# architector1324/micro-raytracer

Hardware: AMD Instinct MI355X
Metric: Msamples/sec (res x spp) (higher is better)
Workload: dtype f32

## Files before the change

### micro_raytracer_amd/csrc/mrt_pack.cpp

```cpp
#include "mrt_pack.h"

#include <math.h>
#include <stdarg.h>
#include <stdio.h>
#include <string.h>

#include <algorithm>
#include <map>
#include <array>

namespace mrt {
namespace {

constexpr u32 kBvhMinInstances = 24;

struct H3 { float x, y, z; };
inline H3 h3(float x, float y, float z) { H3 r = {x, y, z}; return r; }
inline H3 hadd(H3 a, H3 b) { return h3(a.x + b.x, a.y + b.y, a.z + b.z); }
inline H3 hsub(H3 a, H3 b) { return h3(a.x - b.x, a.y - b.y, a.z - b.z); }
inline H3 hmuls(H3 a, float s) { return h3(a.x * s, a.y * s, a.z * s); }
inline H3 hneg(H3 a) { return h3(-a.x, -a.y, -a.z); }
inline H3 hhadam(H3 a, H3 b) { return h3(a.x * b.x, a.y * b.y, a.z * b.z); }
inline float hdot(H3 a, H3 b) { return a.x * b.x + a.y * b.y + a.z * b.z; }
inline H3 hcross(H3 a, H3 b) { return h3(a.y * b.z - a.z * b.y, a.z * b.x - a.x * b.z, a.x * b.y - a.y * b.x); }
// ... 683 lines not shown
    if (!ident) {
        double M[9];
        for (int a = 0; a < 3; ++a) for (int b2 = 0; b2 < 3; ++b2) { double acc = 0; for (int k = 0; k < 3; ++k) acc += (double)X[XF_R + a * 3 + k] * X[XF_L + k * 3 + b2]; M[a * 3 + b2] = acc; }
        for (int a = 0; a < 3 && ortho; ++a) for (int b2 = 0; b2 < 3; ++b2) { double acc = 0; for (int k = 0; k < 3; ++k) acc += M[a * 3 + k] * M[b2 * 3 + k]; if (!(fabs(acc - (a == b2 ? 1.0 : 0.0)) < 1e-4)) ortho = false; }
        for (int a = 0; a < 3; ++a) { lo[a] = -rad; hi[a] = rad; }
    }
    const double pp[3] = {pos.x, pos.y, pos.z};
    bd.ok = ortho && rad < 1e6;
    for (int a = 0; a < 3 && bd.ok; ++a) {
        const double slack = 1e-3 * fmax(fabs(lo[a]), fabs(hi[a])) + 1e-6;
        bd.mn[a] = (float)(pp[a] + lo[a] - slack); bd.mx[a] = (float)(pp[a] + hi[a] + slack);
        if (!(fabs(pp[a]) < 1e6) || !(bd.mn[a] <= bd.mx[a])) bd.ok = false;
    }
    return bd;
}

int add_instance(const mrt_renderer &o, u32 r, const mrt_instance &in, Tables &T, std::string &err)
{
    u32 ir[INST_WORDS] = {0};
    u32 ix[INSTX_WORDS] = {0};
    const H3 pos = h3(in.pos[0], in.pos[1], in.pos[2]);
    put3(ir + INST_POS, pos);
    const u32 xf = T.xf_of(in.dir);
    if ((unsigned long long)xf * XF_WORDS >= (1ull << 28)) return reject(err, MRT_ERR_LIMIT, "too many distinct instance directions");
    const float *X = T.xf_tab.data() + (size_t)xf * XF_WORDS;
    ir[INST_TAG] = o.kind | (bits(X[XF_IDENT]) ? TAG_IDENT : 0u) | ((xf * XF_WORDS) << TAG_XF_SHIFT);
    ix[INSTX_REND] = r;
    const u32 *geo = &T.rend_tab[(size_t)r * REND_WORDS + REND_GEO];
    if (o.kind == MRT_KIND_SPHERE) {
        ir[INST_P3] = geo[0];
    } else if (o.kind == MRT_KIND_PLANE) {
        const H3 nn = h3(fbits(geo[0]), fbits(geo[1]), fbits(geo[2])), nraw = h3(fbits(geo[3]), fbits(geo[4]), fbits(geo[5]));
        ir[INST_P3] = bits(hdot(hneg(nn), pos));
        ir[INST_P5] = geo[0]; ir[INST_P5 + 1] = geo[1]; ir[INST_P5 + 2] = geo[2];
        put3(ix + INSTX_PLANE_NW, hnorm(mul3(X + XF_R, mul3(X + XF_L, nraw))));
    } else if (o.kind == MRT_KIND_BOX) {
        ir[INST_P3] = geo[0]; ir[INST_P5] = geo[1]; ir[INST_P5 + 1] = geo[2];
    }
    T.inst_tab.insert(T.inst_tab.end(), ir, ir + INST_WORDS);
    T.instx_tab.insert(T.instx_tab.end(), ix, ix + INSTX_WORDS);
    const bool tri = o.kind == MRT_KIND_TRIANGLE;
    T.bounds.push_back(instance_bound(o.kind, o.param, tri ? o.param : o.tris, tri ? 3 : (size_t)o.n_tris * 3, X, pos));
    return MRT_OK;
}

bool build_inst_bvh(Tables &T)
{
    std::vector<u32> elig;
    for (u32 i = 0; i < T.n_inst(); ++i) (T.bounds[i].ok ? elig : T.lin_list).push_back(i);
    if (T.n_inst() < kBvhMinInstances || elig.size() < kBvhMinInstances / 2) { T.lin_list.clear(); return false; }
    std::vector<TriBox> ib(T.n_inst());
    for (u32 i : elig) for (int a = 0; a < 3; ++a) { const Bound &b = T.bounds[i]; ib[i].mn[a] = b.mn[a]; ib[i].mx[a] = b.mx[a]; ib[i].c[a] = 0.5f * b.mn[a] + 0.5f * b.mx[a]; }
    TbvhBuild build{ib, T.bvh_nodes, T.bvh_inst, MRT_IBVH_LEAF_MAX};
    build.make(elig, 0, elig.size());
    const u32 n_nodes = (u32)(T.bvh_nodes.size() / BVH_WORDS);
    for (u32 k = 0; k < n_nodes; ++k) { float *q = T.bvh_nodes.data() + (size_t)k * BVH_WORDS; if (bits(q[BVH_SKIP]) >= n_nodes) q[BVH_SKIP] = fbits(BVH_END); }
    return true;
}

bool all_ident(const Tables &T)
{
    bool all = T.n_inst() > 0;
    const u32 xf0 = all ? T.inst_tab[INST_TAG] >> TAG_XF_SHIFT : 0u;
    for (u32 i = 0; i < T.n_inst() && all; ++i) {
        const u32 tag = T.inst_tab[(size_t)i * INST_WORDS + INST_TAG];
        all = (tag & TAG_IDENT) != 0u && memcmp(&T.xf_tab[tag >> TAG_XF_SHIFT], &T.xf_tab[xf0], XF_IDENT * sizeof(float)) == 0;
    }
    return all;
}

bool axis_table(Tables &T, bool plain_ident)
{
    bool scan = plain_ident;
    for (u32 i = 0; i < T.n_inst() && scan; ++i) {
        const u32 *ir = &T.inst_tab[(size_t)i * INST_WORDS];
        const u32 kind = ir[INST_TAG] & TAG_KIND_MASK;
        auto bounded = [](u32 w) { return fabsf(fbits(w)) <= kAxisMax; };
        u32 code = 0u, sd = 0u;
        bool ok = bounded(ir[INST_POS]) && bounded(ir[INST_POS + 1]) && bounded(ir[INST_POS + 2]) && bounded(ir[INST_P3]);
        if (kind == KIND_PLANE) {
            u32 ones = 0u, zeros = 0u;
            for (u32 k = 0; k < 3u; ++k) {
                const u32 w = ir[INST_P5 + k], mag = w & 0x7fffffffu;
                if (mag == 0x3f800000u) { ++ones; code = k + 1u; sd = ir[INST_P3] ^ (w & 0x80000000u); }
                else if (mag == 0u) ++zeros;
            }
            ok = ok && ones == 1u && zeros == 2u;
        } else if (kind != KIND_SPHERE) ok = false;
        T.axis_tab.push_back(code); T.axis_tab.push_back(sd);
        scan = ok;
    }
    return scan;
}

void inst_margins(const Tables &T, Params &P)
{
    float r_min = 3.0e38f;
    bool sphere = false;
    for (u32 i : T.bvh_inst) {
        if ((T.inst_tab[(size_t)i * INST_WORDS + INST_TAG] & TAG_KIND_MASK) != KIND_SPHERE) continue;
        sphere = true;
        for (int a = 0; a < 3; ++a) r_min = std::min(r_min, 0.5f * (T.bounds[i].mx[a] - T.bounds[i].mn[a]));
    }
    P.inst_k = 1e-4f;
    P.inst_ksq = !sphere ? 0.0f : (r_min > 1e-12f ? 4e-6f / r_min : 1e30f);
    P.inst_kpos = sphere ? 1e-5f : 2e-6f;
}

int check_lights(const mrt_scene &sc, std::string &err)
{
    for (u32 l = 0; l < sc.n_light; ++l) if (sc.light[l].kind > MRT_LIGHT_DIR) return reject(err, MRT_ERR_SCENE, "unknown light kind");
    return MRT_OK;
}

int level_order_wide(Tables &T, std::string &err)
{
    struct Ref { u32 depth, mesh, local; };
    std::vector<Ref> order;
    std::vector<std::vector<u32>> newi(T.wide.size());
    for (size_t m = 0; m < T.wide.size(); ++m) { newi[m].resize(T.wide[m].size()); for (size_t k = 0; k < T.wide[m].size(); ++k) order.push_back({T.wide[m][k].depth, (u32)m, (u32)k}); }
    std::stable_sort(order.begin(), order.end(), [](const Ref &a, const Ref &b) { return a.depth < b.depth; });
    if (order.size() >= (1u << 24)) return reject(err, MRT_ERR_LIMIT, "triangle BVHs too large");
    for (size_t k = 0; k < order.size(); ++k) newi[order[k].mesh][order[k].local] = (u32)k;
    T.tbvh_tab.assign(order.size() * B4_WORDS, 0.0f);
    for (size_t k = 0; k < order.size(); ++k) {
        const Wide4 &w = T.wide[order[k].mesh][order[k].local];
        float *q = T.tbvh_tab.data() + k * B4_WORDS;
        for (int c = 0; c < 4; ++c) {
            q[B4_CX + c] = w.c[c][0]; q[B4_CY + c] = w.c[c][1]; q[B4_CZ + c] = w.c[c][2];
            q[B4_HX + c] = w.h[c][0]; q[B4_HY + c] = w.h[c][1]; q[B4_HZ + c] = w.h[c][2];
            u32 cw = w.child[c];
            if (cw & B4_INTERNAL) cw = B4_INTERNAL | newi[order[k].mesh][cw & ~B4_INTERNAL];
            q[B4_CHILD + c] = fbits(cw);
        }
    }
    for (size_t m = 0; m < T.wide.size(); ++m) T.mesh_tab[(size_t)T.wide_mesh[m] * MESH_WORDS + MESH_TBVH] = newi[m][0];
    return MRT_OK;
}

int emit(const mrt_scene &sc, const mrt_env *env, const Tables &T, Packed &out, std::string &err)
{
    Params &P = out.P;
    Blob B;
    P.n_rend = sc.n_renderer; P.n_inst = T.n_inst(); P.n_light = sc.n_light;
    P.n_lin = (u32)T.lin_list.size(); P.n_bvh_nodes = (u32)(T.bvh_nodes.size() / BVH_WORDS);
    out.n_lin = P.n_lin; out.n_bvh_nodes = P.n_bvh_nodes;
    P.off_rend = B.table(T.rend_tab);
    P.off_cam = B.align4(); B.put(P.cam_L, 9); B.put(P.cam_R, 9);
    P.off_lin = B.table(T.lin_list);
    P.off_bvh = B.table(T.bvh_nodes);
    P.off_bvhinst = B.table(T.bvh_inst);
    P.off_inst = B.table(T.inst_tab);
    P.off_instx = B.table(T.instx_tab);
    P.off_axis = 0u; P.axis_scan = out.axis_scan ? 1u : 0u;
    if (out.axis_scan) P.off_axis = B.table(T.axis_tab);
    P.off_xf = B.table(T.xf_tab);
    P.off_mat = B.table(T.mat_tab);
    P.off_light = B.align4();
    for (u32 l = 0; l < sc.n_light; ++l) {
        const mrt_light &li = sc.light[l];
        B.u(li.kind);
        if (li.kind == MRT_LIGHT_POINT) B.f3(h3(li.v[0], li.v[1], li.v[2]));
        else B.f3(hnorm(hneg(hnorm(h3(li.v[0], li.v[1], li.v[2])))));
        B.f(li.pwr);
        B.f3(h3(li.color[0], li.color[1], li.color[2]));
    }
    P.off_tex = B.align4();
    B.w.resize(B.w.size() + (size_t)sc.n_textures * TEX_WORDS, 0);
    P.off_lut = B.align4();
    for (int k = 0; k < 256; ++k) B.f((float)k / 255.0f);
    P.off_mesh = B.table(T.mesh_tab);
    P.off_node = B.table(T.node_tab);
    P.off_parent = B.table(T.parent_tab);
    P.off_tbvh = B.table(T.tbvh_tab);
// ... 86 lines not shown
```

### micro_raytracer_amd/csrc/mrt_scene.h

```cpp
#pragma once
#include <stddef.h>

#include "mrt_math.h"

namespace mrt {

constexpr u32 REND_WORDS = 16;
constexpr u32 INST_WORDS = 8;
constexpr u32 XF_WORDS = 20;
constexpr u32 MAT_WORDS = 16;
constexpr u32 LIGHT_WORDS = 8;
constexpr u32 TEX_WORDS = 4;
constexpr u32 MESH_WORDS = 12;
constexpr u32 TRI_WORDS = 9;
constexpr u32 NODE_WORDS = 8;

enum : u32 { REND_KIND = 0, REND_INST_OFF = 1, REND_INST_CNT = 2, REND_FLAGS = 3, REND_GEO = 4 };
enum : u32 { RF_HAS_MAPS = 1u, RF_HAS_UV = 2u, RF_HAS_VN = 4u };
enum : u32 { REND_VATTR = 15 };
constexpr u32 VATTR_WORDS = 16;
enum : u32 { VATTR_VN = 0, VATTR_UV = 9 };

enum : u32 { INST_POS = 0, INST_P3 = 3, INST_TAG = 4, INST_P5 = 5 };
enum : u32 { INSTX_REND = 0, INSTX_PLANE_NW = 1 };
constexpr u32 INSTX_WORDS = 4;
enum : u32 { AXIS_CODE = 0, AXIS_SD = 1 };
constexpr u32 AXIS_WORDS = 2;
constexpr float kAxisMax = 0x1p38f;
constexpr u32 TAG_KIND_MASK = 7u, TAG_IDENT = 8u, TAG_XF_SHIFT = 4u;

enum : u32 { XF_L = 0, XF_R = 9, XF_IDENT = 18 };

enum : u32 { MAT_ALBEDO = 0, MAT_ROUGH = 3, MAT_METAL = 4, MAT_GLASS = 5, MAT_OPACITY = 6, MAT_EMIT = 7, MAT_MAP = 8, MAT_FLAGS = 14 };
enum : u32 { MATF_BILINEAR = 1u, MATF_CLAMP_V = 2u };
enum : u32 { MAP_TEX = 0, MAP_ROUGH = 1, MAP_METAL = 2, MAP_GLASS = 3, MAP_OPACITY = 4, MAP_EMIT = 5 };

enum : u32 { LIGHT_KIND = 0, LIGHT_V = 1, LIGHT_PWR = 4, LIGHT_COLOR = 5 };

enum : u32 { TEX_W = 0, TEX_H = 1, TEX_OFF = 2, TEX_FMT = 3 };
enum : u32 { TEXFMT_NONE = 0, TEXFMT_F32 = 1, TEXFMT_U8 = 2 };

enum : u32 { ENV_W = 0, ENV_H = 1, ENV_OFF = 2, ENV_FMT = 3, ENV_MAP = 4, ENV_ROT = 5, ENV_PWR = 6, ENV_FLAGS = 7 };
enum : u32 { ENVF_BILINEAR = 1u };
constexpr u32 ENV_WORDS = 8;
enum : u32 { ENVMAP_SPHERE = 0, ENVMAP_LATLONG = 1 };

enum : u32 { MESH_TRI0 = 0, MESH_NTRI = 1, MESH_ROOT = 2, MESH_LEAF0 = 3, MESH_TBVH = 4, MESH_NIDS = 5, MESH_BC = 6, MESH_BH = 9 };
constexpr u32 NO_NODE = 0xffffffffu;

enum : u32 { NODE_HALF = 0, NODE_REL = 3, NODE_FIRST = 6, NODE_COUNT = 7 };

constexpr u32 B4_WORDS = 28;
constexpr u32 B4_INTERNAL = 0x80000000u;
constexpr u32 kWalkCapMin = 8u, kWalkCapMax = 16u, kWalkCapDefault = 16u;
enum : u32 { B4_CX = 0, B4_CY = 4, B4_CZ = 8, B4_HX = 12, B4_HY = 16, B4_HZ = 20, B4_CHILD = 24 };
constexpr u32 BVH_WORDS = 8;
constexpr u32 MEMB_SLOT_BITS = 22u, MEMB_SLOT_MASK = (1u << MEMB_SLOT_BITS) - 1u;
enum : u32 { BVH_C = 0, BVH_H = 3, BVH_SKIP = 6, BVH_LEAF = 7 };
constexpr u32 BVH_END = 0xffffffffu;

enum : u32 { KIND_SPHERE = 0, KIND_PLANE = 1, KIND_BOX = 2, KIND_TRIANGLE = 3, KIND_MESH = 4 };
enum : u32 { LK_POINT = 0, LK_DIR = 1 };

constexpr u32 kChunk = 16;

struct Params {
    u32 nw, nh;
    u32 local_rows, shard_index, shard_count, shard_rows;
    u32 n_samples, sample_base;
    u32 k_split;
    u32 to_planes;
    u32 seed_lo, seed_hi;
    u32 bounce;
    float q;
    float w, h, aspect;
    float inv2tan;
    float cam_pos[3];
    float aprt, foc;
    float cam_L[9], cam_R[9];
    u32 cam_ident;
    float sky[3];
    float sky_init[3];
    u32 n_rend, n_light, n_inst;
    u32 n_lin, n_bvh_nodes;
    float inst_ksq;
    float inst_k, inst_kpos;
    u32 off_lin, off_bvh, off_bvhinst;
    u32 off_cam;
    u32 off_rend, off_inst, off_instx, off_xf, off_mat, off_light, off_tex, off_lut, off_mesh, off_tri, off_node, off_leaf;
    u32 off_tbvh, off_memb, off_membe, off_parent;
    u32 n_tbvh_hot;
    u32 walk_cap;
    u32 blob_words;
    u32 lds_words;
    u32 lds_words_warm;
    u32 lds_words_hot;
    u32 tiles_x, tiles_y;
    u32 count_segments;
    const u32 *blob;
    float *accum;
    float *partial;
    unsigned long long partial_stride;
    unsigned long long *segments;
    u32 *tile_counter;
    u32 persist_grid;
    u32 off_env;
    u32 off_axis;
    u32 axis_scan;
};
static_assert(sizeof(Params) % 8 == 0 && offsetof(Params, axis_scan) + 4 == sizeof(Params), "Params has no tail padding");

// ... 25 lines not shown
```

### micro_raytracer_amd/csrc/mrt_trace.h

```cpp
#pragma once
#include "mrt_scene.h"

namespace mrt {

#ifndef MRT_UNIFORM_TAG
#define MRT_UNIFORM_TAG 1
#endif
#ifndef MRT_T0_FROM_KEY
#define MRT_T0_FROM_KEY 1
#endif
#ifndef MRT_NZFIN_PRODUCT
#define MRT_NZFIN_PRODUCT 1
#endif
#ifndef MRT_SHADOW_QUEUE
#define MRT_SHADOW_QUEUE 0
#endif
#ifndef MRT_LEAF_QUEUE
#define MRT_LEAF_QUEUE 8u
#endif
constexpr u32 kLeafQueue = MRT_LEAF_QUEUE;

#ifndef MRT_PROBE
#define MRT_PROBE(phase)
#endif
#ifndef MRT_COUNT
#define MRT_COUNT(counter)
#endif
#ifndef MRT_PROBE_INST
#define MRT_PROBE_INST(i)
#endif
#if defined(MRT_PHASE_TIMING) && defined(__HIP_DEVICE_COMPILE__)
#define MRT_TICK(slot) do { const unsigned long long now_ = __builtin_amdgcn_s_memtime(); phase_ticks[slot] += now_ - phase_last; phase_last = now_; } while (0)
#define MRT_TICK_DECL unsigned long long phase_ticks[4] = {0ull, 0ull, 0ull, 0ull}; unsigned long long phase_last = __builtin_amdgcn_s_memtime()
#define MRT_TICK_OUT(dst) do { for (int k_ = 0; k_ < 4; ++k_) (dst)[k_] = phase_ticks[k_]; } while (0)
#else
#define MRT_TICK(slot)
#define MRT_TICK_DECL
#define MRT_TICK_OUT(dst)
#endif
#ifndef MRT_PROBE_FALLBACK
#define MRT_PROBE_FALLBACK(ro, rd, dd)
#endif
#ifndef MRT_PROBE_ROUND
#define MRT_PROBE_ROUND(steps, tris, membs)
#endif
enum : u32 { CT_TRACE = 0, CT_LIN_TEST, CT_BVH_NODE, CT_BVH_TEST, CT_MESH_CALL, CT_MESH_ROOT_HIT, CT_TBVH_NODE, CT_TBVH_TRI, CT_TBVH_TRI_HIT, CT_MEMB_BOX, CT_TRACE_ANY, CT_WALK_OVERFLOW, CT_WALK_ROUND, CT_REF_TRI, CT_REF_BOX, CT_AXIS_SCAN, CT_COUNT };
enum : u32 { PH_ITER = 0, PH_REGEN, PH_SPHERE_MATH, PH_PLANE_HIT, PH_SHADE, PH_NORMAL_NONPLANE, PH_SCATTER1, PH_SCATTER2, PH_REFRACT, PH_EMIT_END, PH_LIGHTS, PH_COUNT };

constexpr float kE = 0.0001f;
constexpr float kBig = 1.0f / 0.0001f;

struct V3 { float x, y, z; };
MRT_HD V3 v3(float x, float y, float z) { V3 r; r.x = x; r.y = y; r.z = z; return r; }
MRT_HD V3 add(V3 a, V3 b) { return v3(a.x + b.x, a.y + b.y, a.z + b.z); }
MRT_HD V3 sub(V3 a, V3 b) { return v3(a.x - b.x, a.y - b.y, a.z - b.z); }
MRT_HD float dot(V3 a, V3 b) { return a.x * b.x + a.y * b.y + a.z * b.z; }
MRT_HD V3 muls(V3 a, float s) { return v3(a.x * s, a.y * s, a.z * s); }
MRT_HD V3 neg(V3 a) { return v3(-a.x, -a.y, -a.z); }
MRT_HD V3 hadam(V3 a, V3 b) { return v3(a.x * b.x, a.y * b.y, a.z * b.z); }
MRT_HD V3 cross(V3 a, V3 b) { return v3(a.y * b.z - a.z * b.y, a.z * b.x - a.x * b.z, a.x * b.y - a.y * b.x); }
MRT_HD float mag(V3 a) { return sqrt_(a.x * a.x + a.y * a.y + a.z * a.z); }
MRT_HD V3 norm(V3 a) { return muls(a, recip_sqrt_(a.x * a.x + a.y * a.y + a.z * a.z)); }
MRT_HD V3 reflect(V3 d, V3 n) { return sub(d, muls(n, 2.0f * dot(d, n))); }
MRT_HD V3 m3mul(const float *m, V3 v)
{
    return v3(m[0] * v.x + m[1] * v.y + m[2] * v.z, m[3] * v.x + m[4] * v.y + m[5] * v.z, m[6] * v.x + m[7] * v.y + m[8] * v.z);
}
MRT_HD V3 ld3(const float *F, u32 i) { return v3(F[i], F[i + 1], F[i + 2]); }
struct alignas(16) F4 { float x, y, z, w; };
MRT_HD F4 ld4(const float *F, u32 i) { return *reinterpret_cast<const F4 *>(F + i); }
MRT_HD u32 ldu(const float *F, u32 i) { return f2u(F[i]); }
struct alignas(8) F2 { float x, y; };
MRT_HD F2 ld2(const float *F, u32 i) { return *reinterpret_cast<const F2 *>(F + i); }

MRT_HD bool nzfin(float x)
{
#if defined(__HIP_DEVICE_COMPILE__)
    return __builtin_amdgcn_classf(x, 0x198);
#else
    const float a = fabs_(x);
    return a > 0.0f && a < kInf;
#endif
}
MRT_HD bool nzfin3(V3 v) { return nzfin(v.x) && nzfin(v.y) && nzfin(v.z); }
MRT_HD bool nzfin3_product(V3 v) { return MRT_NZFIN_PRODUCT ? nzfin((v.x * v.y) * v.z) : nzfin3(v); }
MRT_HD u32 mul24(u32 a, u32 b)
{
    return (a & 0xffffffu) * (b & 0xffffffu);
}
MRT_HD void sched_fence()
{
#if defined(__HIP_DEVICE_COMPILE__)
    __builtin_amdgcn_sched_barrier(0);
#endif
}
MRT_HD u32 opaque_v(u32 x)
{
#if defined(__HIP_DEVICE_COMPILE__)
    asm volatile("" : "+v"(x));
#endif
    return x;
}
MRT_HD u32 opaque_s(u32 x)
{
#if defined(__HIP_DEVICE_COMPILE__)
    asm volatile("" : "+s"(x));
#endif
    return x;
}
MRT_HD u32 lowest_bit(u32 x) { return (u32)__builtin_ctz(x | 0x80000000u); }

MRT_HD V3 xf_full(const float *X, V3 v) { return m3mul(X + XF_R, m3mul(X + XF_L, v)); }
MRT_HD V3 xf_vec(const float *X, bool ident, V3 v)
{
    if (ident && nzfin3_product(v)) return v;
    return xf_full(X, v);
}

MRT_HD V3 recip_patched(V3 d)
{
    V3 m;
#if defined(MRT_FAST_IEEE)
    if (wave_all(in_window(d.x) && in_window(d.y) && in_window(d.z))) {
        m = v3(div_core_(1.0f, d.x, rcp_refined_(d.x)), div_core_(1.0f, d.y, rcp_refined_(d.y)), div_core_(1.0f, d.z, rcp_refined_(d.z)));
        return m;
    }
#endif
    m = v3(1.0f / d.x, 1.0f / d.y, 1.0f / d.z);
    if (fabs_(m.x) == kInf) m.x = kBig;
// ... 607 lines not shown
        }
        for (;;) {
            u32 leaf_a = 0u, leaf_b = 0u;
            u32 probe_steps = 0, probe_membs = 0; (void)probe_steps; (void)probe_membs;
            bool walking = node != BVH_END;
            while (walking) {
                ++probe_steps;
                const F4 na = ld4(B0, node * BVH_WORDS), nb = ld4(B0, node * BVH_WORDS + 4);
                MRT_COUNT(CT_TBVH_NODE);
                const u32 skip = f2u(nb.z);
                const u32 leaf = f2u(nb.w), child = node + 1u;
                const bool hit = cull_hit(R, na.x, na.y, na.z, na.w, nb.x, nb.y);
                const u32 cand = hit ? leaf : 0u;
                const bool have_a = leaf_a != 0u;
                leaf_b |= have_a ? cand : 0u;
                leaf_a |= have_a ? 0u : cand;
                node = hit ? child : skip;
                walking = node != BVH_END && leaf_b == 0u;
            }
            if (leaf_a == 0u) { MRT_PROBE_ROUND(probe_steps, 0u, 0u); break; }
            const u32 cnt_a = leaf_a >> 24, first_a = leaf_a & 0xffffffu, cnt_b = leaf_b >> 24, first_b = leaf_b & 0xffffffu;
            MRT_PROBE_ROUND(probe_steps, cnt_a + cnt_b, 0u);
            for (u32 j = 0; j < cnt_a + cnt_b; ++j) {
                const u32 id = j < cnt_a ? first_a + j : first_b + (j - cnt_a);
                const float *T = CT + P.off_tri + (tri0 + id) * TRI_WORDS;
                float t;
                MRT_COUNT(CT_TBVH_TRI);
                if (!tri_isect(add(ld3(T, 0), pos), ld3(T, 3), ld3(T, 6), ro, rd, t)) continue;
                MRT_COUNT(CT_TBVH_TRI_HIT);
                u32 sl, sh;
                if (!memb_candidate<ANY>(S, C, tri0, root, id, ro, m, pos, sl, sh)) continue;
                if (ANY) return true;
                tri_take(best, t, id, sl, sh, t0, i0, t1, i1);
            }
        }
        return best.any;
    }

    count_fallback(P, 7);
    MRT_PROBE_FALLBACK(ro, rd, dd);
    return mesh_isect_ref<ANY, FEAT>(S, mesh, ro, rd, m, pos, t0, i0, t1, i1);
}

#if defined(__HIP_DEVICE_COMPILE__)
MRT_HD u32 wave_uniform(u32 v) { return (u32)__builtin_amdgcn_readfirstlane((int)v); }
#else
MRT_HD u32 wave_uniform(u32 v) { return v; }
#endif
template <bool ANY, u32 FEAT, bool UNIFORM = false>
MRT_HD bool isect_instance(const Scn &S, const RayPre &ray, u32 i, const F4 &ia, const F4 &ib, float &t0, float &t1, i32 &i0, i32 &i1, const float *X0 = nullptr)
{
    const float *F = S.U;
    const Params &P = *S.P;
    const V3 pos = v3(ia.x, ia.y, ia.z);
    const u32 tag = (UNIFORM && (FEAT & F_TRI) && MRT_UNIFORM_TAG) ? wave_uniform(f2u(ib.x)) : f2u(ib.x);
    const u32 kind = (UNIFORM && (FEAT & F_IDENT)) ? wave_uniform(tag & TAG_KIND_MASK) : (tag & TAG_KIND_MASK);
    const bool ident = (FEAT & F_IDENT) ? true : (tag & TAG_IDENT) != 0;
    const float *X = (FEAT & F_IDENT) ? X0 : F + P.off_xf + (tag >> TAG_XF_SHIFT);
    const V3 ro = add(pos, xf_vec(X, ident, sub(ray.o, pos)));
    const bool fast_d = (FEAT & F_IDENT) ? true : (ident && ray.d_ok);
    V3 rd = ray.d, m = ray.m;
    float dd = ray.dd;
    if (!fast_d) {
        rd = xf_full(X, ray.d);
        if constexpr (FEAT & F_BOX) m = recip_patched(rd);
        dd = dot(rd, rd);
    }
    t0 = 0.0f; t1 = 0.0f; i0 = -1; i1 = -1;
    if (kind == KIND_SPHERE) return sphere_isect(ia.w, sub(ro, pos), rd, dd, t0, t1);
    if (kind == KIND_PLANE) { const bool h = plane_isect(v3(ib.y, ib.z, ib.w), ia.w, ro, rd, t0); t1 = t0; return h; }
    if ((FEAT & F_BOX) && kind == KIND_BOX) return box_isect(v3(ia.w, ib.y, ib.z), ro, m, pos, t0, t1);
    if (FEAT & F_TRI) {
        const float *R = F + P.off_rend + ldu(F, P.off_instx + i * INSTX_WORDS + INSTX_REND) * REND_WORDS;
        if (kind == KIND_TRIANGLE) {
            const bool h = tri_isect(add(ld3(R, REND_GEO), pos), ld3(R, REND_GEO + 3), ld3(R, REND_GEO + 6), ro, rd, t0);
            t1 = t0;
            return h;
        }
        if ((FEAT & F_BOX) && kind == KIND_MESH) return mesh_isect<ANY, FEAT>(S, ldu(R, REND_GEO), ro, rd, dd, m, pos, t0, i0, t1, i1);
    }
    return false;
}

template <bool V> struct BoolTag { static constexpr bool value = V; };

template <bool ANY, u32 FEAT>
MRT_HD bool trace(const Scn &S, const RayPre &ray_, Hit &best)
{
    const float *F = S.U;
    const Params &P = *S.P;
    i32 best_key = 0x7fffffff;
    best.rend = -1; best.inst = 0; best.t0 = 0.0f; best.t1 = 0.0f; best.i0 = -1; best.i1 = -1;
    const float *I = F + P.off_inst;

    if (ANY) { MRT_COUNT(CT_TRACE_ANY); } else { MRT_COUNT(CT_TRACE); }
    const float *X0 = nullptr;
    RayPre ray_i = ray_;
    if constexpr (FEAT & F_IDENT) {
        X0 = F + P.off_xf + (ldu(I, INST_TAG) >> TAG_XF_SHIFT);
        if (!ray_.d_ok) {
            ray_i.d = xf_full(X0, ray_.d);
            if constexpr (FEAT & F_BOX) ray_i.m = recip_patched(ray_i.d);
            ray_i.dd = dot(ray_i.d, ray_i.d);
        }
    }
    const RayPre &ray = ray_i;
    auto consider = [&](u32 i, const F4 &ia, const F4 &ib, auto in_order, auto uniform) -> bool {
        float t0, t1;
        MRT_COUNT(CT_LIN_TEST);
        MRT_PROBE_INST(i);
        i32 i0, i1;
        if (!isect_instance<ANY, FEAT, decltype(uniform)::value>(S, ray, i, ia, ib, t0, t1, i0, i1, X0)) return false;
        if (ANY) return true;
        const i32 key = total_key(t0);
        const unsigned long long pair = ((unsigned long long)((u32)key ^ 0x80000000u) << 32) | i;
        const unsigned long long best_pair = ((unsigned long long)((u32)best_key ^ 0x80000000u) << 32) | (best.rend < 0 ? 0xffffffffu : best.inst);
        const bool better = decltype(in_order)::value ? key < best_key : pair < best_pair;
        if (better) {
            best_key = key;
            best.rend = 0; best.inst = i; best.t1 = t1; best.i0 = i0; best.i1 = i1;
            if constexpr ((FEAT & F_BVH) != 0 || !MRT_T0_FROM_KEY) best.t0 = t0;
        }
        return false;
    };
    using InOrder = BoolTag<(FEAT & F_BVH) == 0>;
    using AnyOrder = BoolTag<false>;
    using Shared = BoolTag<true>;
    using PerLane = BoolTag<false>;

    const bool bvh = (FEAT & F_BVH) != 0;
    const u32 n = bvh ? P.n_lin : P.n_inst;
    bool scanned = false;
    if constexpr (!ANY && FEAT == F_IDENT && MRT_T0_FROM_KEY) {
        const V3 o = ray_.o, d = ray_.d;
        const bool tame = (int)in_window(d.x) & (int)in_window(d.y) & (int)in_window(d.z) & (int)(fabs_(o.x) <= kAxisMax) & (int)(fabs_(o.y) <= kAxisMax) &
                          (int)(fabs_(o.z) <= kAxisMax);
        if (P.axis_scan && n && wave_all(tame)) {
            scanned = true;
            MRT_COUNT(CT_AXIS_SCAN);
            const float *A = F + P.off_axis;
#if defined(MRT_FAST_IEEE)
            const V3 r = v3(rcp_refined_(d.x), rcp_refined_(d.y), rcp_refined_(d.z));
#else
            const V3 r = v3(0.0f, 0.0f, 0.0f);
#endif
            auto plane = [&](u32 i, float ok, float dk, float rk, float pk, float sd) {
                const float ro = pk + (ok - pk);
                const float num = -(ro + sd);
                float tt;
#if defined(MRT_FAST_IEEE)
                if (wave_all(fabs_(num) >= kWinLo)) tt = div_core_(num, dk, rk);
                else
#endif
                    tt = num / dk;
                (void)rk;
                const i32 kb = (i32)f2u(tt);
                if (kb > 0 && kb < best_key) { best_key = kb; best.inst = i; best.t1 = tt; }
            };
            auto test = [&](u32 i, const F4 &ia, const F2 &ax) {
                MRT_COUNT(CT_LIN_TEST);
                MRT_PROBE_INST(i);
                const u32 code = wave_uniform(f2u(ax.x));
                if (code == 1u) plane(i, o.x, d.x, r.x, ia.x, ax.y);
                else if (code == 2u) plane(i, o.y, d.y, r.y, ia.y, ax.y);
                else if (code == 3u) plane(i, o.z, d.z, r.z, ia.z, ax.y);
                else {
                    const V3 pos = v3(ia.x, ia.y, ia.z);
                    const V3 ro = add(pos, sub(o, pos));
                    float t0 = 0.0f, t1 = 0.0f;
                    if (sphere_isect(ia.w, sub(ro, pos), d, ray_.dd, t0, t1)) {
                        const i32 key = total_key(t0);
                        if (key < best_key) { best_key = key; best.inst = i; best.t1 = t1; }
                    }
                }
            };
            u32 j = 0;
            F4 a0 = ld4(I, 0), b0 = a0;
            F2 c0 = ld2(A, 0), e0 = c0;
            for (;;) {
                if (j + 1u < n) { b0 = ld4(I, (j + 1u) * INST_WORDS); e0 = ld2(A, (j + 1u) * AXIS_WORDS); }
                test(j, a0, c0);
                if (++j >= n) break;
                if (j + 1u < n) { a0 = ld4(I, (j + 1u) * INST_WORDS); c0 = ld2(A, (j + 1u) * AXIS_WORDS); }
                test(j, b0, e0);
                if (++j >= n) break;
            }
            best.rend = best_key != 0x7fffffff ? 0 : -1;
        }
    }
    if (scanned) {
    } else if (!bvh && !(FEAT & F_TRI) && n) {
        u32 j = 0;
        F4 a0 = ld4(I, 0), a1 = ld4(I, 4), b0 = a0, b1 = a1;
        for (;;) {
            if (j + 1u < n) { b0 = ld4(I, (j + 1u) * INST_WORDS); b1 = ld4(I, (j + 1u) * INST_WORDS + 4); }
            if (consider(j, a0, a1, InOrder(), Shared())) return true;
            if (++j >= n) break;
            if (j + 1u < n) { a0 = ld4(I, (j + 1u) * INST_WORDS); a1 = ld4(I, (j + 1u) * INST_WORDS + 4); }
            if (consider(j, b0, b1, InOrder(), Shared())) return true;
            if (++j >= n) break;
        }
    } else if (n) {
        const float *Lst = F + P.off_lin;
        u32 cur = bvh ? ldu(Lst, 0) : 0u;
        F4 qa = ld4(I, cur * INST_WORDS), qb = ld4(I, cur * INST_WORDS + 4);
        for (u32 j = 0; j < n; ++j) {
            const F4 ia = qa, ib = qb;
            const u32 i = cur;
            if (j + 1 < n) {
                cur = bvh ? ldu(Lst, j + 1) : j + 1;
                qa = ld4(I, cur * INST_WORDS); qb = ld4(I, cur * INST_WORDS + 4);
            }
            if (consider(i, ia, ib, InOrder(), Shared())) return true;
        }
    }

    if constexpr (bvh) {
        const bool cull = cull_ok(ray_.o, ray_.dd);
        CullRay R = cull_ray(ray_.d);
        const float *N0 = F + P.off_bvh;
        u32 node = P.n_bvh_nodes ? 0u : BVH_END;
        float mg;
        {
            const F4 ra = ld4(N0, 0), rb = ld4(N0, 4);
            const V3 r = sub(v3(ra.x, ra.y, ra.z), ray_.o);
            const float ext = fmax_(fmax_(fabs_(r.x) + ra.w, fabs_(r.y) + rb.x), fabs_(r.z) + rb.y);
            const float obig = fmax_(fmax_(fabs_(ray_.o.x), fabs_(ray_.o.y)), fabs_(ray_.o.z));
            const float ksq = fmin_(P.inst_ksq * ext, 4e-3f) * MRT_MARGIN_SCALE;
            mg = fma_fast(P.inst_k * MRT_MARGIN_SCALE + ksq, ext, fma_fast(P.inst_kpos * MRT_MARGIN_SCALE, obig + obig + ext, 1e-6f * MRT_MARGIN_SCALE));
        }
        cull_from(R, ray_.o, mg);
        for (;;) {
            u32 leaf_a = 0u, leaf_b = 0u;
            bool walking = node != BVH_END;
            const float far = (!ANY && best.rend >= 0 && best.t0 >= 0.0f) ? best.t0 + 1e-3f * best.t0 + mg : kInf;
            while (walking) {
                const F4 na = ld4(N0, node * BVH_WORDS), nb = ld4(N0, node * BVH_WORDS + 4);
                MRT_COUNT(CT_BVH_NODE);
                const u32 skip = f2u(nb.z), leaf = f2u(nb.w);
                float tn;
                bool hit_node = cull_hit(R, na.x, na.y, na.z, na.w, nb.x, nb.y, tn);
                if (!ANY) hit_node = hit_node && !(tn > far);
                hit_node = hit_node || !cull;
                const u32 cand = hit_node ? leaf : 0u;
                const bool have_a = leaf_a != 0u;
                leaf_b |= have_a ? cand : 0u;
                leaf_a |= have_a ? 0u : cand;
                node = (hit_node && leaf == 0u) ? node + 1u : skip;
                walking = node != BVH_END && leaf_b == 0u;
            }
            if (leaf_a == 0u) break;
            const u32 cnt_a = leaf_a >> 24, first_a = leaf_a & 0xffffffu, cnt_b = leaf_b >> 24, first_b = leaf_b & 0xffffffu;
            for (u32 k = 0; k < cnt_a + cnt_b; ++k) {
                const u32 i = ldu(F, P.off_bvhinst + (k < cnt_a ? first_a + k : first_b + (k - cnt_a)));
                if (consider(i, ld4(I, i * INST_WORDS), ld4(I, i * INST_WORDS + 4), AnyOrder(), PerLane())) return true;
            }
        }
    }
    if (best.rend < 0) return false;
    if constexpr ((FEAT & F_BVH) == 0 && MRT_T0_FROM_KEY) {
        const i32 k = best_key;
        best.t0 = u2f((u32)(k ^ (i32)(((u32)(k >> 31)) >> 1)));
    }
    best.rend = (i32)ldu(S.F, P.off_instx + best.inst * INSTX_WORDS + INSTX_REND);
    return true;
}
// ... 485 lines not shown
```

Before: 10000.

## Streamline axis-aligned scan: inline sphere test, hoist plane guards, pad axis table

The axis-aligned scan path now decides once per wave whether ray origins are away from near-zero values. With that guard in place, the per-plane wave_all window check is dropped in favour of a direct fast divide. The sphere test is inlined with a precomputed reciprocal of 2a and an early reject for rays pointing away. The axis table gets a padding entry so prefetch loads need no bounds branch, and compiler barriers keep the plane arms as separate scalar branches. The packer also rejects planes whose offset is tiny but nonzero, which could send more scenes to the slower generic path. A standalone single-instantiation compile unit is added for inspecting the generated assembly.

```diff
diff --git a/micro_raytracer_amd/csrc/mrt_asm_one.hip b/micro_raytracer_amd/csrc/mrt_asm_one.hip
--- /dev/null
+++ b/micro_raytracer_amd/csrc/mrt_asm_one.hip
@@ -0,0 +1,37 @@
+#include <hip/hip_runtime.h>
+
+#include "mrt_kernels.h"
+#include "mrt_megakernel.h"
+#include "mrt_post.h"
+#include "mrt_trace.h"
+
+#ifndef MRT_ONE_INST
+#define MRT_ONE_INST F_IDENT
+#endif
+#ifndef MRT_ONE_THREADS
+#define MRT_ONE_THREADS 256
+#endif
+#ifndef MRT_ONE_LDS
+#define MRT_ONE_LDS 1
+#endif
+
+namespace mrt {
+
+#undef MRT_SHAPES_64
+#undef MRT_SHAPES_256
+#undef MRT_SHAPES_512
+#undef MRT_SHAPES_1024
+#undef MRT_SHAPES_L2
+#define MRT_SHAPES_64
+#define MRT_SHAPES_256
+#define MRT_SHAPES_512
+#define MRT_SHAPES_1024
+#define MRT_SHAPES_L2
+
+#define MRT_PT_LIST 0
+#include "mrt_pt_kernel.h"
+#undef MRT_PT_LIST
+
+template __global__ void pt_megakernel<MRT_ONE_LDS != 0, MRT_ONE_THREADS, (MRT_ONE_INST)>(const Params, const u32 *__restrict__);
+
+}
diff --git a/micro_raytracer_amd/csrc/mrt_pack.cpp b/micro_raytracer_amd/csrc/mrt_pack.cpp
--- a/micro_raytracer_amd/csrc/mrt_pack.cpp
+++ b/micro_raytracer_amd/csrc/mrt_pack.cpp
@@ -789,7 +789,11 @@
             u32 ones = 0u, zeros = 0u;
             for (u32 k = 0; k < 3u; ++k) {
                 const u32 w = ir[INST_P5 + k], mag = w & 0x7fffffffu;
-                if (mag == 0x3f800000u) { ++ones; code = k + 1u; sd = ir[INST_P3] ^ (w & 0x80000000u); }
+                if (mag == 0x3f800000u) {
+                    ++ones; code = k + 1u; sd = ir[INST_P3] ^ (w & 0x80000000u);
+                    const float pk = fabsf(fbits(ir[INST_POS + k]));
+                    ok = ok && (pk == 0.0f || pk >= kAxisPlaneMin);
+                }
                 else if (mag == 0u) ++zeros;
             }
             ok = ok && ones == 1u && zeros == 2u;
@@ -797,6 +801,7 @@
         T.axis_tab.push_back(code); T.axis_tab.push_back(sd);
         scan = ok;
     }
+    for (u32 k = 0; k < AXIS_WORDS; ++k) T.axis_tab.push_back(0u);
     return scan;
 }
 
diff --git a/micro_raytracer_amd/csrc/mrt_scene.h b/micro_raytracer_amd/csrc/mrt_scene.h
--- a/micro_raytracer_amd/csrc/mrt_scene.h
+++ b/micro_raytracer_amd/csrc/mrt_scene.h
@@ -27,6 +27,7 @@
 enum : u32 { AXIS_CODE = 0, AXIS_SD = 1 };
 constexpr u32 AXIS_WORDS = 2;
 constexpr float kAxisMax = 0x1p38f;
+constexpr float kAxisPlaneMin = 0x1p-15f;
 constexpr u32 TAG_KIND_MASK = 7u, TAG_IDENT = 8u, TAG_XF_SHIFT = 4u;
 
 enum : u32 { XF_L = 0, XF_R = 9, XF_IDENT = 18 };
diff --git a/micro_raytracer_amd/csrc/mrt_trace.h b/micro_raytracer_amd/csrc/mrt_trace.h
--- a/micro_raytracer_amd/csrc/mrt_trace.h
+++ b/micro_raytracer_amd/csrc/mrt_trace.h
@@ -44,7 +44,7 @@
 #ifndef MRT_PROBE_ROUND
 #define MRT_PROBE_ROUND(steps, tris, membs)
 #endif
-enum : u32 { CT_TRACE = 0, CT_LIN_TEST, CT_BVH_NODE, CT_BVH_TEST, CT_MESH_CALL, CT_MESH_ROOT_HIT, CT_TBVH_NODE, CT_TBVH_TRI, CT_TBVH_TRI_HIT, CT_MEMB_BOX, CT_TRACE_ANY, CT_WALK_OVERFLOW, CT_WALK_ROUND, CT_REF_TRI, CT_REF_BOX, CT_AXIS_SCAN, CT_COUNT };
+enum : u32 { CT_TRACE = 0, CT_LIN_TEST, CT_BVH_NODE, CT_BVH_TEST, CT_MESH_CALL, CT_MESH_ROOT_HIT, CT_TBVH_NODE, CT_TBVH_TRI, CT_TBVH_TRI_HIT, CT_MEMB_BOX, CT_TRACE_ANY, CT_WALK_OVERFLOW, CT_WALK_ROUND, CT_REF_TRI, CT_REF_BOX, CT_AXIS_SCAN, CT_AXIS_REDO, CT_COUNT };
 enum : u32 { PH_ITER = 0, PH_REGEN, PH_SPHERE_MATH, PH_PLANE_HIT, PH_SHADE, PH_NORMAL_NONPLANE, PH_SCATTER1, PH_SCATTER2, PH_REFRACT, PH_EMIT_END, PH_LIGHTS, PH_COUNT };
 
 constexpr float kE = 0.0001f;
@@ -818,6 +818,14 @@
     return false;
 }
 
+#if defined(__HIP_DEVICE_COMPILE__)
+#define MRT_ARM_END(name) asm volatile("; axis scan: end of arm " name)
+#define MRT_FORGET_SCALAR(v) asm volatile("" : "+s"(v))
+#else
+#define MRT_ARM_END(name)
+#define MRT_FORGET_SCALAR(v)
+#endif
+
 template <bool V> struct BoolTag { static constexpr bool value = V; };
 
 template <bool ANY, u32 FEAT>
@@ -871,9 +879,16 @@
         const V3 o = ray_.o, d = ray_.d;
         const bool tame = (int)in_window(d.x) & (int)in_window(d.y) & (int)in_window(d.z) & (int)(fabs_(o.x) <= kAxisMax) & (int)(fabs_(o.y) <= kAxisMax) &
                           (int)(fabs_(o.z) <= kAxisMax);
+        auto off0 = [](float x) { return (int)(x == 0.0f) | (int)(fabs_(x) >= kWinLo); };
+        const bool near0 = !(off0(o.x) & off0(o.y) & off0(o.z));
+        bool axis = false;
         if (P.axis_scan && n && wave_all(tame)) {
+            MRT_COUNT(CT_AXIS_SCAN);
+            axis = wave_all(!near0);
+            if (!axis) { MRT_COUNT(CT_AXIS_REDO); }
+        }
+        if (axis) {
             scanned = true;
-            MRT_COUNT(CT_AXIS_SCAN);
             const float *A = F + P.off_axis;
 #if defined(MRT_FAST_IEEE)
             const V3 r = v3(rcp_refined_(d.x), rcp_refined_(d.y), rcp_refined_(d.z));
@@ -883,41 +898,69 @@
             auto plane = [&](u32 i, float ok, float dk, float rk, float pk, float sd) {
                 const float ro = pk + (ok - pk);
                 const float num = -(ro + sd);
-                float tt;
 #if defined(MRT_FAST_IEEE)
-                if (wave_all(fabs_(num) >= kWinLo)) tt = div_core_(num, dk, rk);
-                else
-#endif
-                    tt = num / dk;
+                const float tt = div_core_(num, dk, rk);
+#else
+                const float tt = num / dk;
+#endif
                 (void)rk;
                 const i32 kb = (i32)f2u(tt);
                 if (kb > 0 && kb < best_key) { best_key = kb; best.inst = i; best.t1 = tt; }
             };
+            const float a = ray_.dd, den = 2.0f * a;
+            const bool a_mid = (int)(a > 0.0f) & (int)(a < 1e18f);
+#if defined(MRT_FAST_IEEE)
+            const bool den_ok = in_window(den);
+            const float rden = rcp_refined_(den);
+#endif
+            auto sphere = [&](u32 i, const F4 &ia) {
+                const V3 pos = v3(ia.x, ia.y, ia.z);
+                const V3 ro = add(pos, sub(o, pos));
+                const V3 oo = sub(ro, pos);
+                const float b = 2.0f * dot(oo, d);
+                const float c = dot(oo, oo) - ia.w;
+                const float disc = b * b - 4.0f * a * c;
+                if (disc < 0.0f) return;
+                if (b > 1e-20f && a_mid && disc >= 0.0f) return;
+                MRT_PROBE(PH_SPHERE_MATH);
+#if defined(MRT_FAST_IEEE)
+                const float sqc = sqrt_core_(disc);
+                const float m0 = -b - sqc, m1 = -b + sqc;
+                const float least = __builtin_fminf(__builtin_fminf(disc, fabs_(m0)), fabs_(m1));
+                const float most = __builtin_fmaxf(__builtin_fmaxf(disc, fabs_(m0)), fabs_(m1));
+                if (wave_all((int)(least >= kWinLo) & (int)(most <= kWinHi) & (int)den_ok)) {
+                    const float q0 = div_core_(m0, den, rden), q1 = div_core_(m1, den, rden);
+                    const i32 kb = (i32)f2u(q0);
+                    if (kb > 0 && kb < best_key) { best_key = kb; best.inst = i; best.t1 = q1; }
+                    return;
+                }
+#endif
+                const float sq = __builtin_sqrtf(disc);
+                const float q0 = (-b - sq) / den, q1 = (-b + sq) / den;
+                if (q0 < 0.0f) return;
+                const i32 key = total_key(q0);
+                if (key < best_key) { best_key = key; best.inst = i; best.t1 = q1; }
+            };
             auto test = [&](u32 i, const F4 &ia, const F2 &ax) {
                 MRT_COUNT(CT_LIN_TEST);
                 MRT_PROBE_INST(i);
-                const u32 code = wave_uniform(f2u(ax.x));
-                if (code == 1u) plane(i, o.x, d.x, r.x, ia.x, ax.y);
-                else if (code == 2u) plane(i, o.y, d.y, r.y, ia.y, ax.y);
-                else if (code == 3u) plane(i, o.z, d.z, r.z, ia.z, ax.y);
-                else {
-                    const V3 pos = v3(ia.x, ia.y, ia.z);
-                    const V3 ro = add(pos, sub(o, pos));
-                    float t0 = 0.0f, t1 = 0.0f;
-                    if (sphere_isect(ia.w, sub(ro, pos), d, ray_.dd, t0, t1)) {
-                        const i32 key = total_key(t0);
-                        if (key < best_key) { best_key = key; best.inst = i; best.t1 = t1; }
-                    }
-                }
+                u32 code = wave_uniform(f2u(ax.x));
+                if (code == 1u) { plane(i, o.x, d.x, r.x, ia.x, ax.y); MRT_ARM_END("x"); }
+                MRT_FORGET_SCALAR(code);
+                if (code == 2u) { plane(i, o.y, d.y, r.y, ia.y, ax.y); MRT_ARM_END("y"); }
+                MRT_FORGET_SCALAR(code);
+                if (code == 3u) { plane(i, o.z, d.z, r.z, ia.z, ax.y); MRT_ARM_END("z"); }
+                MRT_FORGET_SCALAR(code);
+                if (code == 0u) { sphere(i, ia); MRT_ARM_END("sphere"); }
             };
             u32 j = 0;
-            F4 a0 = ld4(I, 0), b0 = a0;
-            F2 c0 = ld2(A, 0), e0 = c0;
+            F4 a0 = ld4(I, 0), b0;
+            F2 c0 = ld2(A, 0), e0;
             for (;;) {
-                if (j + 1u < n) { b0 = ld4(I, (j + 1u) * INST_WORDS); e0 = ld2(A, (j + 1u) * AXIS_WORDS); }
+                b0 = ld4(I, (j + 1u) * INST_WORDS); e0 = ld2(A, (j + 1u) * AXIS_WORDS);
                 test(j, a0, c0);
                 if (++j >= n) break;
-                if (j + 1u < n) { a0 = ld4(I, (j + 1u) * INST_WORDS); c0 = ld2(A, (j + 1u) * AXIS_WORDS); }
+                a0 = ld4(I, (j + 1u) * INST_WORDS); c0 = ld2(A, (j + 1u) * AXIS_WORDS);
                 test(j, b0, e0);
                 if (++j >= n) break;
             }
```

After: 10520, median of 6. 1.05x the previous value.
